# su1phurd/UAV-WRF-LES-PPO-LSTM

Hardware: AMD Instinct MI355X
Metric: env-steps/sec (rollout + GAE + 5-epoch PPO update), 4096 envs x 128 T per GPU, LSTM h=128 x1 (higher is better)
Workload: dtype f32

## Files before the change

uav-wrf-les-ppo-lstm_amd/csrc/common.h:

```cpp
#pragma once
#include <hip/hip_runtime.h>
#include <stdint.h>
#include <stdio.h>
#include <stdlib.h>
#include <string.h>
#include "../../include/uavppo.h"

struct uav_form_table {
    struct { const void* p; int v; } e[8];
    int next;
    void record(const void* p, int v) {
        for (auto& x : e)
            if (x.p == p) { x.v = v; return; }
        e[next] = {p, v};
        next = (next + 1) % 8;
    }
    int find(const void* p) const {
        for (auto& x : e)
            if (x.p == p) return x.v;
        return -1;
    }
};
struct uav_ctx {
    int device;
    int num_cu;
    void* ws;
    size_t ws_bytes;
    double* pow075;
    double* wave;
    double* ftab;
    int lstm_arith;
    unsigned debug;
    hipStream_t side[3];
    hipEvent_t side_ev[8];
    void* comm;
    int comm_rank, comm_world;
    uav_form_table dg_form;
    uav_form_table hslot_form;
};
static inline void uav_dg_record(uav_ctx* ctx, const void* p, int packed) { ctx->dg_form.record(p, packed); }
static inline int uav_dg_form(const uav_ctx* ctx, const void* p) { return ctx->dg_form.find(p); }

extern thread_local int g_uav_arith;
extern thread_local unsigned g_uav_debug;
static inline bool uav_want_f32_mfma() { return g_uav_arith == UAV_ARITH_F32_MFMA; }
static inline bool uav_want_bf16x6() { return g_uav_arith == UAV_ARITH_BF16X6; }
static inline bool uav_debug(unsigned bit) { return (g_uav_debug & bit) != 0; }
static inline void uav_enter(const struct uav_ctx* ctx);

static inline void uav_enter(const uav_ctx* ctx) {
    g_uav_arith = ctx->lstm_arith;
    g_uav_debug = ctx->debug;
}

void uav_set_error(const char* fmt, ...);

hipError_t uav_dyn_lds(const void* kernel, int bytes);

#define UAV_CHECK_HIP(expr)                                                          \
    do {                                                                             \
        hipError_t e_ = (expr);                                                      \
        if (e_ != hipSuccess) {                                                      \
            uav_set_error("%s:%d: %s -> %s", __FILE__, __LINE__, #expr, hipGetErrorString(e_)); \
            return 1;                                                                \
        }                                                                            \
    } while (0)

#define UAV_REQUIRE(cond, ...)                                                       \
    do {                                                                             \
        if (!(cond)) {                                                               \
            uav_set_error(__VA_ARGS__);                                              \
            return 2;                                                                \
        }                                                                            \
    } while (0)

#define UAV_LAUNCH_CHECK() UAV_CHECK_HIP(hipGetLastError())

static inline hipStream_t as_stream(uav_stream s) { return reinterpret_cast<hipStream_t>(s); }

constexpr int WAVE = 64;
// ... 85 lines not shown
    __device__ __forceinline__ static f32x4 mma(vec a, vec b, f32x4 c) { return __builtin_amdgcn_mfma_f32_16x16x32_bf16(a, b, c, 0, 0, 0); }
    template <class W>
    __device__ __forceinline__ static void gates_slab(f32x4 (&acc)[4], f32x4 (&)[4], W w, const vec (&a)[NP]) {
#pragma unroll
        for (int q = 0; q < 4; ++q) acc[q] = mma(w(q, 0), a[2], acc[q]);
#pragma unroll
        for (int q = 0; q < 4; ++q) acc[q] = mma(w(q, 1), a[1], acc[q]);
#pragma unroll
        for (int q = 0; q < 4; ++q) acc[q] = mma(w(q, 2), a[0], acc[q]);
#pragma unroll
        for (int q = 0; q < 4; ++q) acc[q] = mma(w(q, 0), a[1], acc[q]);
#pragma unroll
        for (int q = 0; q < 4; ++q) acc[q] = mma(w(q, 1), a[0], acc[q]);
#pragma unroll
        for (int q = 0; q < 4; ++q) acc[q] = mma(w(q, 0), a[0], acc[q]);
    }
    template <class W, class B>
    __device__ __forceinline__ static void head_slab(f32x4& ha, f32x4&, W w, B h) {
        ha = mma(w(0), h(2), ha);
        ha = mma(w(1), h(1), ha);
        ha = mma(w(2), h(0), ha);
        ha = mma(w(0), h(1), ha);
        ha = mma(w(1), h(0), ha);
        ha = mma(w(0), h(0), ha);
    }
    template <class V> __device__ __forceinline__ static V sum(V acc, V) { return acc; }
    template <class W>
    __device__ __forceinline__ static void tile_slab(f32x4& a0, f32x4& a1, W w, const vec (&b)[NP]) {
        a0 = mma(w(0), b[2], a0);
        a1 = mma(w(1), b[1], a1);
        a0 = mma(w(2), b[0], a0);
        a1 = mma(w(0), b[1], a1);
        a0 = mma(w(1), b[0], a0);
        a1 = mma(w(0), b[0], a1);
    }
    __device__ __forceinline__ static f32x4 tile_sum(f32x4 a0, f32x4 a1) { return a0 + a1; }
};

struct DgPack {
    static constexpr int H = 256, NS = 4 * H / 32;
    int N, T, NP, RT;
    __host__ __device__ DgPack(int n, int t) : N(n), T(t), NP((n + 63) / 64 * 64), RT(NP / 16) {}
    __host__ __device__ size_t step_halves() const { return (size_t)RT * NS * 1024; }
    __host__ __device__ size_t piece_bytes() const { return (size_t)T * step_halves() * 2; }
    __host__ __device__ size_t bytes() const { return piece_bytes() + 2 * (size_t)T * NP * sizeof(float); }
    __host__ __device__ unsigned short* pieces(void* base, int t) const { return (unsigned short*)base + (size_t)t * step_halves(); }
    __host__ __device__ const unsigned short* pieces(const void* base, int t) const { return (const unsigned short*)base + (size_t)t * step_halves(); }
    __host__ __device__ float* isc(void* base, int t) const { return (float*)((char*)base + piece_bytes()) + (size_t)t * NP; }
    __host__ __device__ const float* isc(const void* base, int t) const { return (const float*)((const char*)base + piece_bytes()) + (size_t)t * NP; }
    __host__ __device__ float* iscm(void* base, int t) const { return isc(base, T) + (size_t)t * NP; }
    __host__ __device__ const float* iscm(const void* base, int t) const { return isc(base, T) + (size_t)t * NP; }
};

__device__ __forceinline__ double wave_sum(double v) {
#pragma unroll
    for (int o = 32; o > 0; o >>= 1) v += __shfl_down(v, o, 64);
    return v;
}
__device__ __forceinline__ float wave_sum(float v) {
#pragma unroll
    for (int o = 32; o > 0; o >>= 1) v += __shfl_down(v, o, 64);
    return v;
}
__device__ __forceinline__ float wave_allsum(float v) {
#pragma unroll
    for (int o = 32; o > 0; o >>= 1) v += __shfl_xor(v, o, 64);
    return v;
}
template <typename T>
__device__ __forceinline__ T block256_sum(T v, T* sm) {
    v = wave_sum(v);
    const int lane = threadIdx.x & 63, w = threadIdx.x >> 6;
    if (lane == 0) sm[w] = v;
    __syncthreads();
    T r = T(0);
    if (threadIdx.x == 0) r = ((sm[0] + sm[1]) + sm[2]) + sm[3];
    __syncthreads();
    return r;
}
```

uav-wrf-les-ppo-lstm_amd/csrc/ctx.hip:

```cpp
#include <stdarg.h>
#include <mutex>
#include <set>
#include <utility>
#include "common.h"

static thread_local char g_err[512] = "";
thread_local int g_uav_arith = 0;
thread_local unsigned g_uav_debug = 0;
int env_init_tables(uav_ctx* ctx);

void uav_set_error(const char* fmt, ...) {
    va_list ap;
    va_start(ap, fmt);
    vsnprintf(g_err, sizeof(g_err), fmt, ap);
    va_end(ap);
}

hipError_t uav_dyn_lds(const void* kernel, int bytes) {
    static std::mutex mu;
    static std::set<std::pair<int, const void*>> done;
    int dev = 0;
    hipError_t e = hipGetDevice(&dev);
    if (e != hipSuccess) return e;
    std::lock_guard<std::mutex> lock(mu);
    if (done.count({dev, kernel})) return hipSuccess;
    e = hipFuncSetAttribute(kernel, hipFuncAttributeMaxDynamicSharedMemorySize, bytes);
    if (e == hipSuccess) done.insert({dev, kernel});
    return e;
}

extern "C" {

int uav_abi_version(void) { return UAV_ABI_VERSION; }
const char* uav_last_error(void) { return g_err; }

int uav_create(uav_ctx** out, int device, size_t ws_bytes) {
    UAV_REQUIRE(out != nullptr, "uav_create: out is NULL");
    UAV_REQUIRE(ws_bytes >= (1u << 20), "uav_create: ws_bytes must be >= 1 MiB");
    UAV_CHECK_HIP(hipSetDevice(device));
    hipDeviceProp_t prop;
    UAV_CHECK_HIP(hipGetDeviceProperties(&prop, device));
    UAV_REQUIRE(strncmp(prop.gcnArchName, "gfx950", 6) == 0,
                "libuavppo is built for gfx950 (MI355X) only; device %d is %s", device, prop.gcnArchName);
    uav_ctx* c = new uav_ctx();
    c->device = device;
    c->num_cu = prop.multiProcessorCount;
    c->ws_bytes = ws_bytes;
    c->pow075 = nullptr;
    c->wave = nullptr;
    c->ftab = nullptr;
    c->comm = nullptr;
    c->comm_rank = -1;
    c->comm_world = 0;
    c->lstm_arith = getenv("UAV_LSTM_F32_MFMA") ? UAV_ARITH_F32_MFMA : (getenv("UAV_LSTM_BF16X6") ? UAV_ARITH_BF16X6 : UAV_ARITH_FP16X3);
    c->debug = (getenv("UAV_LSTM_STEP_F32") ? UAV_DEBUG_STEP_F32 : 0u) | (getenv("UAV_LSTM_X_F32") ? UAV_DEBUG_X_F32 : 0u) |
               (getenv("UAV_LSTM_DG_F32") ? UAV_DEBUG_DG_F32 : 0u);
    if (hipMalloc(&c->ws, ws_bytes) != hipSuccess) {
        (void)hipFree(c->ws);
        delete c;
        uav_set_error("uav_create: hipMalloc(%zu) failed", ws_bytes);
        return 1;
    }
    if (env_init_tables(c) != 0) {
        (void)hipFree(c->ws);
        (void)hipFree(c->pow075);
        (void)hipFree(c->wave);
        (void)hipFree(c->ftab);
        delete c;
        return 1;
    }
    *out = c;
    return 0;
}

int uav_set_lstm_arith(uav_ctx* ctx, int mode) {
    UAV_REQUIRE(ctx && mode >= UAV_ARITH_FP16X3 && mode <= UAV_ARITH_F32_MFMA, "uav_set_lstm_arith: bad argument");
    ctx->lstm_arith = mode;
    return 0;
}
int uav_get_lstm_arith(const uav_ctx* ctx) { return ctx ? ctx->lstm_arith : -1; }

int uav_set_debug_flags(uav_ctx* ctx, unsigned flags) {
    UAV_REQUIRE(ctx && (flags & ~(UAV_DEBUG_STEP_F32 | UAV_DEBUG_X_F32 | UAV_DEBUG_DG_F32 | UAV_DEBUG_GEMM_TN_OFF)) == 0, "uav_set_debug_flags: bad argument");
    ctx->debug = flags;
    return 0;
}

void uav_destroy(uav_ctx* ctx) {
    if (!ctx) return;
    (void)uav_comm_destroy(ctx);
    for (auto& e : ctx->side_ev)
        if (e) (void)hipEventDestroy(e);
    for (auto& s : ctx->side)
        if (s) (void)hipStreamDestroy(s);
    (void)hipFree(ctx->ws);
    (void)hipFree(ctx->pow075);
    (void)hipFree(ctx->wave);
    (void)hipFree(ctx->ftab);
    delete ctx;
}

}
```

uav-wrf-les-ppo-lstm_amd/csrc/gae.hip:

```cpp
#include "common.h"

__global__ __launch_bounds__(256) void gae_scan_kernel(const float* __restrict__ rew,
                                                       const float* __restrict__ val,
                                                       const float* __restrict__ done,
                                                       const float* __restrict__ last_val, int n_env,
                                                       int T, float gamma, float gl, int mode,
                                                       float* __restrict__ adv) {
#pragma clang fp contract(off)
    const int lane = threadIdx.x & 63;
    const int env = blockIdx.x * 4 + (threadIdx.x >> 6);
    if (env >= n_env) return;
    const size_t row = (size_t)env * T;
    const int nchunk = (T + 63) >> 6;
    float carry = 0.f;
    float v_right = 0.f, d_right = 0.f;
    for (int c = nchunk - 1; c >= 0; --c) {
        const int t = c * 64 + lane;
        const bool in = t < T;
        const float r = in ? rew[row + t] : 0.f;
        const float v = in ? val[row + t] : 0.f;
        const float d = in ? done[row + t] : 0.f;
        float v1 = __shfl_down(v, 1, 64);
        float d1 = __shfl_down(d, 1, 64);
        if (lane == 63) { v1 = v_right; d1 = d_right; }
        float a = 1.f, b = 0.f;
        if (in) {
            float nnt, nv;
            const bool last = (t == T - 1);
            if (mode == UAV_GAE_REFERENCE_EXACT) {
                nnt = 1.0f - (last ? d : d1);
                nv = (last ? v : v1) * nnt;
            } else {
                nnt = 1.0f - d;
                nv = (last ? (last_val ? last_val[env] : 0.f) : v1) * nnt;
            }
            b = (r + gamma * nv) - v;
            a = gl * nnt;
        }
#pragma unroll
        for (int o = 1; o < 64; o <<= 1) {
            const float a2 = __shfl_down(a, o, 64);
            const float b2 = __shfl_down(b, o, 64);
            if (lane + o < 64) {
                b = b + a * b2;
                a = a * a2;
            }
        }
        const float A = b + a * carry;
        if (in) adv[row + t] = A;
        carry = __shfl(A, 0, 64);
        v_right = __shfl(v, 0, 64);
        d_right = __shfl(d, 0, 64);
    }
}

constexpr int STATS_BLOCKS = 512;

__global__ __launch_bounds__(256) void adv_stats_partial(const float* __restrict__ x, int64_t n,
                                                         double* __restrict__ partial) {
    __shared__ double sm[4];
    double s = 0.0, q = 0.0;
    for (int64_t i = (int64_t)blockIdx.x * 256 + threadIdx.x; i < n; i += (int64_t)gridDim.x * 256) {
        const double v = (double)x[i];
        s += v;
        q += v * v;
    }
    s = block256_sum(s, sm);
    q = block256_sum(q, sm);
    if (threadIdx.x == 0) {
        partial[2 * blockIdx.x] = s;
        partial[2 * blockIdx.x + 1] = q;
    }
}

__global__ __launch_bounds__(256) void adv_stats_final(const double* __restrict__ partial, int nb,
                                                       int64_t n, double* __restrict__ stats3) {
    __shared__ double sm[4];
    double s = 0.0, q = 0.0;
    for (int i = threadIdx.x; i < nb; i += 256) {
        s += partial[2 * i];
        q += partial[2 * i + 1];
    }
    s = block256_sum(s, sm);
    q = block256_sum(q, sm);
    if (threadIdx.x == 0) {
        stats3[0] = s;
        stats3[1] = q;
        stats3[2] = (double)n;
    }
}

__global__ __launch_bounds__(256) void adv_normalise_kernel(const float* __restrict__ adv,
                                                            const float* __restrict__ val, int64_t n,
                                                            const double* __restrict__ stats3,
                                                            float* __restrict__ adv_out,
                                                            float* __restrict__ ret_out) {
#pragma clang fp contract(off)
    const double cnt = stats3[2];
    const double mean_d = stats3[0] / cnt;
    const double var = (stats3[1] - cnt * mean_d * mean_d) / (cnt - 1.0);
    const float mean = (float)mean_d;
    float sd = (float)sqrt(var > 0.0 ? var : (var == var ? 0.0 : var));
    if (sd < 1e-6f || sd != sd) sd = 1.0f;
    const float den = sd + 1e-6f;
    for (int64_t i = (int64_t)blockIdx.x * 256 + threadIdx.x; i < n; i += (int64_t)gridDim.x * 256) {
        const float a = (adv[i] - mean) / den;
        adv_out[i] = a;
        ret_out[i] = a + val[i];
    }
}

__global__ __launch_bounds__(1024) void pack_success_kernel(const uint8_t* __restrict__ flags, int64_t n, int cap,
                                                            uint8_t* __restrict__ msg) {
    __shared__ int part[32];
    const int tid = threadIdx.x;
    int64_t per = (n + 1023) / 1024;
    per = (per + 15) / 16 * 16;
    const int64_t lo = (int64_t)tid * per, hi = (lo + per < n) ? lo + per : n;
    const bool vec = (reinterpret_cast<uintptr_t>(flags) & 15) == 0;
    auto visit = [&](auto&& f) {
        int64_t i = lo;
        if (vec)
            for (; i + 16 <= hi; i += 16) {
                const uint4 w = *reinterpret_cast<const uint4*>(flags + i);
                if ((w.x | w.y | w.z | w.w) == 0u) continue;
                const unsigned ww[4] = {w.x, w.y, w.z, w.w};
#pragma unroll
                for (int q = 0; q < 4; ++q)
#pragma unroll
                    for (int k = 0; k < 4; ++k) {
                        const uint8_t v = (ww[q] >> (8 * k)) & 255;
                        if (v) f(v);
                    }
            }
// ... 120 lines not shown
                    succ += __popcll(__ballot(i < n && chunk[k + i] != 0));
                }
                k += n;
                const double env_radius = s.radius;
                s.episodes += n; s.successes += succ;
                s.hist_len += n; s.win_succ += succ;
                const bool full = s.hist_len >= CUR_WINDOW;
                double rate = 0.0;
                if (full) {
                    rate = (double)s.win_succ / (double)s.hist_len;
                    s.bonus = s.bonus * pow(CUR_DECAY_FACTOR, 1.0 + rate);
                    s.bonus_is_f64 = 1.0;
                }
                s.bonus = fmax(s.bonus, 0.1);
                if (full) {
                    if (rate > CUR_SUCCESS_THRESHOLD)
                        s.radius = fmax(CUR_MIN_RADIUS, s.radius * pow(CUR_RADIUS_DECAY, 2.0 + 3.0 * (rate - CUR_SUCCESS_THRESHOLD)));
                    else if (rate < 0.25)
                        s.radius = fmin(CUR_INITIAL_RADIUS, s.radius * 1.1);
                    const double d = s.radius - env_radius;
                    if (fabs(d) > 5.0) s.radius = env_radius + 5.0 * (d > 0.0 ? 1.0 : (d < 0.0 ? -1.0 : 0.0));
                    s.hist_len = 0; s.win_succ = 0;
                }
            }
            __syncthreads();
            if (lane == 0) sh = s;
        }
    }
    __syncthreads();
    if (lane == 0) *st = sh;
}

extern "C" {

int uav_gae(uav_ctx* ctx, const float* rew, const float* val, const float* done,
            const float* last_val, int n_env, int horizon, float gamma, float lam, int mode,
            float* adv, uav_stream stream) {
    UAV_REQUIRE(ctx && rew && val && done && adv, "uav_gae: NULL argument");
    UAV_REQUIRE(n_env > 0 && horizon > 0, "uav_gae: n_env=%d horizon=%d", n_env, horizon);
    UAV_REQUIRE(mode == UAV_GAE_REFERENCE_EXACT || mode == UAV_GAE_STANDARD, "uav_gae: mode %d", mode);
    const float gl = (float)((double)gamma * (double)lam);
    const int blocks = (n_env + 3) / 4;
    hipLaunchKernelGGL(gae_scan_kernel, dim3(blocks), dim3(256), 0, as_stream(stream), rew, val, done,
                       last_val, n_env, horizon, gamma, gl, mode, adv);
    UAV_LAUNCH_CHECK();
    return 0;
}

int uav_adv_stats(uav_ctx* ctx, const float* adv, int64_t n, double* stats3, uav_stream stream) {
    UAV_REQUIRE(ctx && adv && stats3 && n > 0, "uav_adv_stats: bad argument");
    int nb = (int)((n + 1023) / 1024);
    if (nb > STATS_BLOCKS) nb = STATS_BLOCKS;
    double* partial = (double*)ctx->ws;
    hipLaunchKernelGGL(adv_stats_partial, dim3(nb), dim3(256), 0, as_stream(stream), adv, n, partial);
    hipLaunchKernelGGL(adv_stats_final, dim3(1), dim3(256), 0, as_stream(stream), partial, nb, n, stats3);
    UAV_LAUNCH_CHECK();
    return 0;
}

int uav_adv_normalise(uav_ctx* ctx, const float* adv, const float* val, int64_t n,
                      const double* stats3, float* adv_out, float* ret_out, uav_stream stream) {
    UAV_REQUIRE(ctx && adv && val && stats3 && adv_out && ret_out && n > 0, "uav_adv_normalise: bad argument");
    int nb = (int)((n + 1023) / 1024);
    if (nb > 2048) nb = 2048;
    hipLaunchKernelGGL(adv_normalise_kernel, dim3(nb), dim3(256), 0, as_stream(stream), adv, val, n, stats3,
                       adv_out, ret_out);
    UAV_LAUNCH_CHECK();
    return 0;
}


int uav_episode_rows(uav_ctx* ctx, const float* rew, const float* info, const uint8_t* flags, int n_env, int T, int env_offset,
                     double* carry, double* rows, int cap, int32_t* count, uav_stream stream) {
    UAV_REQUIRE(ctx && rew && info && flags && carry && rows && count && n_env > 0 && T > 0 && cap > 0, "uav_episode_rows: bad argument");
    hipLaunchKernelGGL(episode_rows_kernel, dim3((n_env + 63) / 64), dim3(64), 0, as_stream(stream), rew, info, flags, n_env, T, env_offset,
                       carry, rows, cap, count);
    UAV_LAUNCH_CHECK();
    return 0;
}

size_t uav_curriculum_state_bytes(void) { return sizeof(CurriculumState); }

int uav_curriculum_init(uav_ctx* ctx, void* state, double radius, double bonus, int bonus_is_f64, uav_stream stream) {
    UAV_REQUIRE(ctx && state && radius > 0.0, "uav_curriculum_init: bad argument");
    hipLaunchKernelGGL(curriculum_init_kernel, dim3(1), dim3(64), 0, as_stream(stream), (CurriculumState*)state, radius, bonus, bonus_is_f64);
    UAV_LAUNCH_CHECK();
    return 0;
}

int uav_curriculum_update(uav_ctx* ctx, void* state, const uint8_t* msgs, int world, int cap, uav_stream stream) {
    UAV_REQUIRE(ctx && state && msgs && world > 0 && cap > 0, "uav_curriculum_update: bad argument");
    hipLaunchKernelGGL(curriculum_update_kernel, dim3(1), dim3(64), 0, as_stream(stream), (CurriculumState*)state, msgs, world, cap);
    UAV_LAUNCH_CHECK();
    return 0;
}

int uav_pack_success_bits(uav_ctx* ctx, const uint8_t* flags, int64_t n, int cap, uint8_t* msg, uav_stream stream) {
    UAV_REQUIRE(ctx && flags && msg && n > 0 && cap > 0, "uav_pack_success_bits: bad argument");
    hipLaunchKernelGGL(pack_success_kernel, dim3(1), dim3(1024), 0, as_stream(stream), flags, n, cap, msg);
    UAV_LAUNCH_CHECK();
    return 0;
}

}
```

uav-wrf-les-ppo-lstm_amd/csrc/loss.hip:

```cpp
#include "common.h"
#include "philox.h"

#include "loss_core.h"

template <int A>
__device__ __forceinline__ void loss_block_epilogue(const LossAcc& a, const float* s_db, double* partial) {
    __shared__ double sm[4];
    const double s_pl = block256_sum(a.pl, sm), s_vl = block256_sum(a.vl, sm);
    const double s_en = block256_sum(a.en, sm), s_nan = block256_sum(a.nan, sm);
    double dbs[A + 1];
#pragma unroll
    for (int k = 0; k <= A; ++k) dbs[k] = block256_sum((double)s_db[k], sm);
    if (threadIdx.x == 0) {
        double* pp = partial + (size_t)LOSS_PSTRIDE * blockIdx.x;
        pp[0] = s_pl; pp[1] = s_vl; pp[2] = s_en; pp[3] = s_nan;
#pragma unroll
        for (int k = 0; k <= A; ++k) pp[4 + k] = dbs[k];
    }
}

template <int A>
__global__ __launch_bounds__(256) void ppo_loss_kernel(
    const float* __restrict__ logits, const float* __restrict__ value, const int32_t* __restrict__ act,
    const float* __restrict__ logp_old, const float* __restrict__ adv, const float* __restrict__ ret,
    const float* __restrict__ val_old, int64_t n, float inv_n, float clip, float beta,
    double* __restrict__ partial, float* __restrict__ dlogits, float* __restrict__ dvalue, int ldl, int ldv) {
    LossAcc acc{0.0, 0.0, 0.0, 0.0};
    float s_db[A + 1];
#pragma unroll
    for (int k = 0; k <= A; ++k) s_db[k] = 0.f;
    for (int64_t i = (int64_t)blockIdx.x * 256 + threadIdx.x; i < n; i += (int64_t)gridDim.x * 256) {
        float z[A], dz[A];
#pragma unroll
        for (int k = 0; k < A; ++k) z[k] = logits[i * ldl + k];
        const float dV = ppo_sample<A>(z, value[i * ldv], act[i], logp_old[i], adv[i], ret[i], val_old[i], inv_n, clip,
                                       beta, acc, dz);
        dvalue[i * ldv] = dV;
        s_db[A] += dV;
#pragma unroll
        for (int k = 0; k < A; ++k) {
            dlogits[i * ldl + k] = dz[k];
            s_db[k] += dz[k];
        }
    }
    loss_block_epilogue<A>(acc, s_db, partial);
}

typedef float f32x4_l __attribute__((ext_vector_type(4)));
template <int A, int H>
__global__ __launch_bounds__(256) void ppo_loss_from_y_kernel(
    const float* __restrict__ y, const float* __restrict__ w_head, const float* __restrict__ b_head,
    const int32_t* __restrict__ act, const float* __restrict__ logp_old, const float* __restrict__ adv,
    const float* __restrict__ ret, const float* __restrict__ val_old, int64_t n, float inv_n, float clip, float beta,
    double* __restrict__ partial, float* __restrict__ dheads) {
    constexpr int KS = H / 4, SEG = KS + 4, S = 4 * SEG + 8, NH = A + 1;
    __shared__ __attribute__((aligned(16))) float wbuf[16 * S];
    __shared__ __attribute__((aligned(16))) float ybuf[4][16 * S];
    __shared__ float hd[4][64 * 9];
    const int lane = threadIdx.x & 63, w = threadIdx.x >> 6, j = lane & 15, kq = lane >> 4;
    for (int idx = threadIdx.x; idx < 16 * H; idx += 256) {
        const int hdx = idx / H, uu = idx % H;
        wbuf[hdx * S + (uu / KS) * SEG + (uu % KS)] = (hdx < NH) ? w_head[(size_t)hdx * H + uu] : 0.f;
    }
    __syncthreads();
    LossAcc acc{0.0, 0.0, 0.0, 0.0};
    float s_db[A + 1];
#pragma unroll
    for (int k = 0; k <= A; ++k) s_db[k] = 0.f;
    float bh[NH];
#pragma unroll
    for (int k = 0; k < NH; ++k) bh[k] = b_head[k];
    const int64_t ntile = (n + 255) / 256;
    for (int64_t tile = blockIdx.x; tile < ntile; tile += gridDim.x) {
        const int64_t row0 = tile * 256 + w * 64;
        f32x4_l c4[4];
#pragma unroll
        for (int mi = 0; mi < 4; ++mi) {
            __builtin_amdgcn_wave_barrier();
#pragma unroll
            for (int i = 0; i < H / 16; ++i) {
                const int idx = i * 64 + lane, row = idx / (H / 4), c = idx % (H / 4);
                const int64_t r = row0 + 16 * mi + row;
                const float4 v = *reinterpret_cast<const float4*>(y + (r < n ? r : n - 1) * H + 4 * c);
                *reinterpret_cast<float4*>(&ybuf[w][row * S + ((4 * c) / KS) * SEG + (4 * c) % KS]) = v;
            }
            __builtin_amdgcn_s_waitcnt(0xc07f);
            __builtin_amdgcn_wave_barrier();
            const float* yr = &ybuf[w][j * S + kq * SEG];
            f32x4_l a0 = {0.f, 0.f, 0.f, 0.f}, a1 = a0;
            const float* wr = wbuf + j * S + kq * SEG;
#pragma unroll
            for (int s = 0; s < KS; s += 4) {
                const float4 av = *reinterpret_cast<const float4*>(yr + s);
                const float4 bv = *reinterpret_cast<const float4*>(wr + s);
                a0 = __builtin_amdgcn_mfma_f32_16x16x4f32(av.x, bv.x, a0, 0, 0, 0);
                a1 = __builtin_amdgcn_mfma_f32_16x16x4f32(av.y, bv.y, a1, 0, 0, 0);
                a0 = __builtin_amdgcn_mfma_f32_16x16x4f32(av.z, bv.z, a0, 0, 0, 0);
                a1 = __builtin_amdgcn_mfma_f32_16x16x4f32(av.w, bv.w, a1, 0, 0, 0);
// ... 69 lines not shown
    const int a = sample_categorical<A>(z, p, u ? &u[i] : nullptr, seed, counter, index_offset + i, forced ? &forced[i] : nullptr, qa, bad);
    if (bad) atomicAdd(nan_count, 1);
    if (probs_out) {
#pragma unroll
        for (int k = 0; k < A; ++k) probs_out[i * A + k] = p[k];
    }
    act_out[i] = a;
    const float lp = logf(fminf(fmaxf(qa, F32_EPS), 1.0f - F32_EPS));
    if (logp_out) logp_out[i] = lp;
    if (act_buf) {
        act_buf[i * T + t] = a;
        logp_buf[i * T + t] = lp;
        val_buf[i * T + t] = logits[i * stride + A];
    }
}

__global__ __launch_bounds__(256) void store_transition_kernel(int n, int T, int t, float* __restrict__ keep,
                                                               const float* __restrict__ rew, const float* __restrict__ done,
                                                               const uint8_t* __restrict__ flags, float* __restrict__ keep_buf,
                                                               float* __restrict__ rew_buf, float* __restrict__ done_buf,
                                                               uint8_t* __restrict__ flags_buf) {
    const int i = blockIdx.x * 256 + threadIdx.x;
    if (i >= n) return;
    const int64_t o = (int64_t)i * T + t;
    const float d = done[i];
    keep_buf[o] = keep[i];
    rew_buf[o] = rew[i];
    done_buf[o] = d;
    flags_buf[o] = flags[i];
    keep[i] = 1.0f - d;
}

int launch_loss_final(double* partial, int nb, int n_heads, double* loss_sums, float* dhead_bias, hipStream_t st) {
    hipLaunchKernelGGL(loss_final_kernel, dim3(1), dim3(1024), 0, st, partial, nb, n_heads, loss_sums, dhead_bias);
    UAV_LAUNCH_CHECK();
    return 0;
}

extern "C" {

int uav_ppo_loss(uav_ctx* ctx, const float* logits, const float* value, const int32_t* act,
                 const float* logp_old, const float* adv, const float* ret, const float* val_old,
                 int64_t n, int n_act, float inv_n, float clip, float ent_beta, double* loss_sums,
                 float* dlogits, float* dvalue, float* dhead_bias, uav_stream stream) {
    UAV_REQUIRE(ctx && logits && act && logp_old && adv && ret && val_old && loss_sums && dlogits,
                "uav_ppo_loss: NULL argument");
    UAV_REQUIRE((value == nullptr) == (dvalue == nullptr), "uav_ppo_loss: value and dvalue must both be NULL (packed) or both given");
    const int ldl = value ? n_act : n_act + 1, ldv = value ? 1 : n_act + 1;
    if (!value) { value = logits + n_act; dvalue = dlogits + n_act; }
    UAV_REQUIRE(n > 0, "uav_ppo_loss: n=%lld", (long long)n);
    int nb = (int)((n + 255) / 256);
    if (nb > LOSS_BLOCKS) nb = LOSS_BLOCKS;
    double* partial = (double*)ctx->ws;
#define LAUNCH_LOSS(A_)                                                                                  \
    hipLaunchKernelGGL(ppo_loss_kernel<A_>, dim3(nb), dim3(256), 0, as_stream(stream), logits, value,   \
                       act, logp_old, adv, ret, val_old, n, inv_n, clip, ent_beta, partial, dlogits, dvalue, ldl, ldv)
    switch (n_act) {
        case 2: LAUNCH_LOSS(2); break;
        case 3: LAUNCH_LOSS(3); break;
        case 4: LAUNCH_LOSS(4); break;
        case 5: LAUNCH_LOSS(5); break;
        case 6: LAUNCH_LOSS(6); break;
        case 8: LAUNCH_LOSS(8); break;
        default: UAV_REQUIRE(false, "uav_ppo_loss: n_act=%d unsupported", n_act);
    }
#undef LAUNCH_LOSS
    hipLaunchKernelGGL(loss_final_kernel, dim3(1), dim3(1024), 0, as_stream(stream), partial, nb, n_act + 1, loss_sums,
                       dhead_bias);
    UAV_LAUNCH_CHECK();
    return 0;
}

int uav_ppo_loss_from_y(uav_ctx* ctx, const float* y, const float* w_head, const float* b_head, const int32_t* act,
                         const float* logp_old, const float* adv, const float* ret, const float* val_old, int64_t n,
                         int hidden, int n_act, float inv_n, float clip, float ent_beta, double* loss_sums, float* dheads,
                         float* dhead_bias, uav_stream stream) {
    UAV_REQUIRE(ctx && y && w_head && b_head && act && logp_old && adv && ret && val_old && loss_sums && dheads,
                "uav_ppo_loss_from_y: NULL argument");
    UAV_REQUIRE(n > 0 && n_act == 5, "uav_ppo_loss_from_y: n=%lld n_act=%d (5 actions supported)", (long long)n, n_act);
    int nb = (int)((n + 255) / 256);
    if (nb > LOSS_BLOCKS) nb = LOSS_BLOCKS;
    double* partial = (double*)ctx->ws;
#define LAUNCH_LY(H_)                                                                                             \
    hipLaunchKernelGGL((ppo_loss_from_y_kernel<5, H_>), dim3(nb), dim3(256), 0, as_stream(stream), y, w_head, b_head, \
                       act, logp_old, adv, ret, val_old, n, inv_n, clip, ent_beta, partial, dheads)
    switch (hidden) {
        case 64: LAUNCH_LY(64); break;
        case 128: LAUNCH_LY(128); break;
        case 256: LAUNCH_LY(256); break;
        default: UAV_REQUIRE(false, "uav_ppo_loss_from_y: hidden=%d unsupported (64/128/256)", hidden);
    }
#undef LAUNCH_LY
    hipLaunchKernelGGL(loss_final_kernel, dim3(1), dim3(1024), 0, as_stream(stream), partial, nb, n_act + 1, loss_sums,
                       dhead_bias);
    UAV_LAUNCH_CHECK();
    return 0;
}

int uav_policy_sample(uav_ctx* ctx, const float* logits, int64_t n, int n_act, const float* u,
                      uint64_t seed, uint64_t counter, int64_t index_offset, const int32_t* forced_act, int32_t* act_out,
                      float* logp_out, float* probs_out, int32_t* nan_count, uav_stream stream) {
    UAV_REQUIRE(ctx && logits && act_out && logp_out && nan_count && n > 0, "uav_policy_sample: bad argument");
    const int nb = (int)((n + 255) / 256);
#define LAUNCH_S(A_)                                                                                      \
    hipLaunchKernelGGL(policy_sample_kernel<A_>, dim3(nb), dim3(256), 0, as_stream(stream), logits, n, u, \
                       seed, counter, index_offset, forced_act, act_out, logp_out, probs_out, nan_count)
    switch (n_act) {
        case 2: LAUNCH_S(2); break;
        case 3: LAUNCH_S(3); break;
        case 4: LAUNCH_S(4); break;
        case 5: LAUNCH_S(5); break;
        case 6: LAUNCH_S(6); break;
        case 8: LAUNCH_S(8); break;
        default: UAV_REQUIRE(false, "uav_policy_sample: n_act=%d unsupported", n_act);
    }
#undef LAUNCH_S
    UAV_LAUNCH_CHECK();
    return 0;
}

int uav_policy_sample_at(uav_ctx* ctx, const float* heads, int64_t heads_stride, int64_t n, int n_act, uint64_t seed,
// ... 37 lines not shown
```

uav-wrf-les-ppo-lstm_amd/csrc/wgrad.hip:

```cpp
#include <stdlib.h>
#include <type_traits>
#include "common.h"

typedef float f32x4 __attribute__((ext_vector_type(4)));

constexpr int KC = 16;

template <int H>
struct WG {
    static constexpr int NW = H / 16;
    static constexpr int NT_ = H / 16 + 1;
    static constexpr int NC = H + 16;
    static constexpr int SG = 4 * H + 16;
    static constexpr int SB = H + 16;
    static constexpr int SY = H + 16;
    static constexpr int SD = 48;
    static constexpr int BUF = KC * (SG + SB + SY + SD);
    static constexpr size_t LDS = 2 * BUF * sizeof(float);
    static constexpr size_t SLAB = (size_t)4 * H * NC + 16 * H;
};

template <int H>
__global__ __launch_bounds__(H * 4) void lstm_wgrad_kernel(
    const float* __restrict__ dgates, const float* __restrict__ y, const float* __restrict__ keep,
// ... 419 lines not shown
    commit_b(0);
    load_b(1);
    split_pair(0, 0);
    lds_barrier();
    WX_PROF_DECL;
    for (int sl = 0; sl < nslab; ++sl) {
        const int buf = sl & 1;
        WX_PROF_MARK(0);
        mfma_pair(buf, 0, sl);
        WX_PROF_DEP(acc[0][NT_ - 1]); WX_PROF_DEP(acc[1][NT_ - 1]); WX_PROF_MARK(2);
        commit_b(buf ^ 1);
        if constexpr (!P::LOADS_BETWEEN_TILES) load_b(sl + 2);
        WX_PROF_MARK(5);
        split_pair(sl, 1);
        WX_PROF_DEP(ap[0][0]); WX_PROF_DEP(ap[1][NP - 1]); WX_PROF_MARK(3);
        mfma_pair(buf, 1, sl);
        WX_PROF_DEP(acc[2][NT_ - 1]); WX_PROF_DEP(acc[3][NT_ - 1]); WX_PROF_MARK(4);
        if (!late) { lds_barrier(); WX_PROF_MARK(7); }
        split_pair(sl + 1, 0);
        WX_PROF_DEP(ap[0][0]); WX_PROF_DEP(ap[1][NP - 1]); WX_PROF_MARK(1);
        if (late) { lds_barrier(); WX_PROF_MARK(7); }
    }
    WX_PROF_FLUSH();
    float* slab = slabs + (size_t)blockIdx.x * WG<H>::SLAB;
#pragma unroll
    for (int mi = 0; mi < 4; ++mi)
#pragma unroll
        for (int r = 0; r < 4; ++r) {
            const float usc = pol.row_unscale(mi, r, kq);
#pragma unroll
            for (int ni = 0; ni < NT_; ++ni)
                slab[(size_t)(64 * w + 32 * (mi >> 1) + 2 * (4 * kq + r) + (mi & 1)) * G::NC + 16 * ni + j] =
                    acc[mi][ni][r] * (ni == NT_ - 1 ? usc * (P::BSCALE / P::XSCALE) : usc);
        }
#pragma unroll
    for (int r = 0; r < 4; ++r) slab[(size_t)4 * H * G::NC + (size_t)(4 * kq + r) * H + 16 * w + j] = acch[r];
}

template <int H, bool HEADS>
__global__ __launch_bounds__(H * 4) void lstm_wgrad_x6_kernel(
    const float* __restrict__ dgates, const float* __restrict__ y, const float* __restrict__ keep,
    const float* __restrict__ h0, const float* __restrict__ x, int I, const float* __restrict__ dheads, int NH,
    int N, int T, int rows_per_block, float* __restrict__ slabs) {
    lstm_wgrad_split<H, HEADS, WgBf16x6>(dgates, y, keep, h0, x, I, dheads, NH, N, T, rows_per_block, slabs);
}
template <int H, bool HEADS>
__global__ __launch_bounds__(H * 4) void lstm_wgrad_h3_kernel(
    const float* __restrict__ dgates, const float* __restrict__ y, const float* __restrict__ keep,
    const float* __restrict__ h0, const float* __restrict__ x, int I, const float* __restrict__ dheads, int NH,
    int N, int T, int rows_per_block, float* __restrict__ slabs) {
    lstm_wgrad_split<H, HEADS, WgF16x3>(dgates, y, keep, h0, x, I, dheads, NH, N, T, rows_per_block, slabs);
}

template <int H>
__global__ __launch_bounds__(256) void wgrad_reduce_kernel(const float* __restrict__ slabs, int nb, int I, int NH,
                                                           float* __restrict__ dw_ih, float* __restrict__ dw_hh,
                                                           float* __restrict__ db, float* __restrict__ db_hh,
                                                           float* __restrict__ dw_head) {
    using G = WG<H>;
    const size_t o = (size_t)blockIdx.x * 256 + threadIdx.x;
    if (o >= G::SLAB) return;
    float p8[8] = {0.f, 0.f, 0.f, 0.f, 0.f, 0.f, 0.f, 0.f};
    int b = 0;
    for (; b + 8 <= nb; b += 8)
#pragma unroll
        for (int k = 0; k < 8; ++k) p8[k] += slabs[(size_t)(b + k) * G::SLAB + o];
    for (; b < nb; ++b) p8[0] += slabs[(size_t)b * G::SLAB + o];
    const float s = ((p8[0] + p8[1]) + (p8[2] + p8[3])) + ((p8[4] + p8[5]) + (p8[6] + p8[7]));
    const size_t gsz = (size_t)4 * H * G::NC;
    if (o < gsz) {
        const int m = (int)(o / G::NC), c = (int)(o % G::NC);
        if (c < H) dw_hh[(size_t)m * H + c] = s;
        else if (c - H < I) dw_ih[(size_t)m * I + (c - H)] = s;
        else if (c - H == 6) {
            db[m] = s;
            if (db_hh) db_hh[m] = s;
        }
    } else if (dw_head) {
        const int a = (int)((o - gsz) / H), uu = (int)((o - gsz) % H);
        if (a < NH) dw_head[(size_t)a * H + uu] = s;
    }
}

template <class P, int H, bool HEADS>
static constexpr auto wgrad_split_kernel() {
    if constexpr (std::is_same<P, WgF16x3>::value) return &lstm_wgrad_h3_kernel<H, HEADS>;
    else return &lstm_wgrad_x6_kernel<H, HEADS>;
}

template <class P, int H>
static int launch_wgrad_split(const float* dgates, const float* y, const float* keep, const float* h0, const float* x, int I,
                              const float* dheads, int NH, int N, int T, int nb, int rpb, float* slabs, hipStream_t st) {
    const auto kern = dheads ? wgrad_split_kernel<P, H, true>() : wgrad_split_kernel<P, H, false>();
    const size_t lds = WGS<H, P>::LDS;
    UAV_CHECK_HIP(uav_dyn_lds(reinterpret_cast<const void*>(kern), (int)lds));
    hipLaunchKernelGGL(kern, dim3(nb), dim3(H * 4), lds, st, dgates, y, keep, h0, x, I, dheads, NH, N, T, rpb, slabs);
    return 0;
}

template <int H>
static int launch_wgrad(uav_ctx* ctx, const float* dgates, const float* y, const float* keep, const float* h0,
                        const float* x, int I, const float* dheads, int NH, int N, int T,
                        float* dw_ih, float* dw_hh, float* db, float* db_hh, float* dw_head, hipStream_t st) {
    using G = WG<H>;
    const int64_t NTr = (int64_t)N * T;
    int nb = ctx->num_cu;
    const int64_t max_nb = (int64_t)(ctx->ws_bytes / (G::SLAB * sizeof(float)));
    if (nb > max_nb) nb = (int)max_nb;
    UAV_REQUIRE(nb >= 1, "uav_lstm_wgrad: workspace too small for one slab");
    int64_t rpb = (NTr + nb - 1) / nb;
    rpb = (rpb + KC - 1) / KC * KC;
    nb = (int)((NTr + rpb - 1) / rpb);
    float* slabs = (float*)ctx->ws;
    {
        int64_t rpx = (NTr + nb - 1) / nb;
        rpx = (rpx + KS6 - 1) / KS6 * KS6;
        const int nbx = (int)((NTr + rpx - 1) / rpx);
        const bool split_ok = (NTr % rpx == 0) && T >= 8 && I <= 6 && (!dheads || NH <= 8) && NTr * 4 * H < (1ll << 30) &&
                              !uav_want_f32_mfma();
        if (split_ok) {
            const int rc = uav_want_bf16x6()
                               ? launch_wgrad_split<WgBf16x6, H>(dgates, y, keep, h0, x, I, dheads, NH, N, T, nbx, (int)rpx, slabs, st)
                               : launch_wgrad_split<WgF16x3, H>(dgates, y, keep, h0, x, I, dheads, NH, N, T, nbx, (int)rpx, slabs, st);
            if (rc) return rc;
            hipLaunchKernelGGL((wgrad_reduce_kernel<H>), dim3((unsigned)((G::SLAB + 255) / 256)), dim3(256), 0, st, slabs,
                               nbx, I, NH, dw_ih, dw_hh, db, db_hh, dw_head);
            UAV_LAUNCH_CHECK();
            return 0;
        }
    }
    UAV_CHECK_HIP(uav_dyn_lds(reinterpret_cast<const void*>(&lstm_wgrad_kernel<H>), (int)G::LDS));
    hipLaunchKernelGGL((lstm_wgrad_kernel<H>), dim3(nb), dim3(H * 4), G::LDS, st, dgates, y, keep, h0, x, I, dheads, NH, N,
                       T, rpb, slabs);
    hipLaunchKernelGGL((wgrad_reduce_kernel<H>), dim3((unsigned)((G::SLAB + 255) / 256)), dim3(256), 0, st, slabs, nb, I,
                       NH, dw_ih, dw_hh, db, db_hh, dw_head);
    UAV_LAUNCH_CHECK();
    return 0;
}

int lstm_wgrad_fused(uav_ctx* ctx, const float* dgates, const float* y, const float* keep, const float* h0,
                     const float* x, int I, const float* dheads, int NH, int N, int T, int H,
                     float* dw_ih, float* dw_hh, float* db, float* db_hh, float* dw_head, hipStream_t st) {
    switch (H) {
        case 64: return launch_wgrad<64>(ctx, dgates, y, keep, h0, x, I, dheads, NH, N, T, dw_ih, dw_hh, db, db_hh, dw_head, st);
        case 128: return launch_wgrad<128>(ctx, dgates, y, keep, h0, x, I, dheads, NH, N, T, dw_ih, dw_hh, db, db_hh, dw_head, st);
    }
    uav_set_error("lstm_wgrad_fused: H=%d unsupported", H);
    return 2;
}
```

Measured before the change: 76.00 million.

## Fuse final reductions via last-block tickets, pack loss I/O, vectorize wgrad reduce

Merges the separate single-block finalize kernels for advantage stats and PPO loss into the partial-reduction kernels, using an atomic last-block ticket so one fewer launch is needed per call. The loss kernel also gains a packed float2 load/store path for contiguous logits+value rows and processes two samples per iteration to raise memory-level parallelism. The wgrad slab reduction now reads float4 and splits the slab dimension across 8 thread groups combined in LDS. This adds atomics, fences and a persistent ticket buffer, which must be reset correctly and cannot be shared by concurrent launches.

```diff
diff --git a/uav-wrf-les-ppo-lstm_amd/csrc/common.h b/uav-wrf-les-ppo-lstm_amd/csrc/common.h
--- a/uav-wrf-les-ppo-lstm_amd/csrc/common.h
+++ b/uav-wrf-les-ppo-lstm_amd/csrc/common.h
@@ -26,6 +26,7 @@
     int num_cu;
     void* ws;
     size_t ws_bytes;
+    unsigned* tickets;
     double* pow075;
     double* wave;
     double* ftab;
@@ -217,6 +218,26 @@
     __host__ __device__ const float* iscm(const void* base, int t) const { return isc(base, T) + (size_t)t * NP; }
 };
 
+enum { UAV_TICKET_LOSS = 0, UAV_TICKET_ADV_STATS = 1, UAV_TICKET_COUNT = 4 };
+__device__ __forceinline__ bool last_block_ticket(unsigned* ticket) {
+    __shared__ int s_last;
+    if (threadIdx.x == 0) {
+        __threadfence();
+        const unsigned t = atomicAdd(ticket, 1u);
+        const bool last = (t == gridDim.x - 1);
+        if (last) __hip_atomic_store(ticket, 0u, __ATOMIC_RELAXED, __HIP_MEMORY_SCOPE_AGENT);
+        s_last = last;
+    }
+    __syncthreads();
+    const bool last = s_last != 0;
+    if (last) __threadfence();
+    return last;
+}
+__device__ __forceinline__ double ld_partial(const double* p) {
+    return __builtin_bit_cast(double, __hip_atomic_load(reinterpret_cast<const unsigned long long*>(p), __ATOMIC_RELAXED,
+                                                        __HIP_MEMORY_SCOPE_AGENT));
+}
+
 __device__ __forceinline__ double wave_sum(double v) {
 #pragma unroll
     for (int o = 32; o > 0; o >>= 1) v += __shfl_down(v, o, 64);
diff --git a/uav-wrf-les-ppo-lstm_amd/csrc/ctx.hip b/uav-wrf-les-ppo-lstm_amd/csrc/ctx.hip
--- a/uav-wrf-les-ppo-lstm_amd/csrc/ctx.hip
+++ b/uav-wrf-les-ppo-lstm_amd/csrc/ctx.hip
@@ -46,6 +46,7 @@
     c->device = device;
     c->num_cu = prop.multiProcessorCount;
     c->ws_bytes = ws_bytes;
+    c->tickets = nullptr;
     c->pow075 = nullptr;
     c->wave = nullptr;
     c->ftab = nullptr;
@@ -61,7 +62,16 @@
         uav_set_error("uav_create: hipMalloc(%zu) failed", ws_bytes);
         return 1;
     }
+    if (hipMalloc(&c->tickets, UAV_TICKET_COUNT * sizeof(unsigned)) != hipSuccess ||
+        hipMemset(c->tickets, 0, UAV_TICKET_COUNT * sizeof(unsigned)) != hipSuccess || hipDeviceSynchronize() != hipSuccess) {
+        (void)hipFree(c->tickets);
+        (void)hipFree(c->ws);
+        delete c;
+        uav_set_error("uav_create: ticket allocation failed");
+        return 1;
+    }
     if (env_init_tables(c) != 0) {
+        (void)hipFree(c->tickets);
         (void)hipFree(c->ws);
         (void)hipFree(c->pow075);
         (void)hipFree(c->wave);
@@ -94,6 +104,7 @@
     for (auto& s : ctx->side)
         if (s) (void)hipStreamDestroy(s);
     (void)hipFree(ctx->ws);
+    (void)hipFree(ctx->tickets);
     (void)hipFree(ctx->pow075);
     (void)hipFree(ctx->wave);
     (void)hipFree(ctx->ftab);
diff --git a/uav-wrf-les-ppo-lstm_amd/csrc/gae.hip b/uav-wrf-les-ppo-lstm_amd/csrc/gae.hip
--- a/uav-wrf-les-ppo-lstm_amd/csrc/gae.hip
+++ b/uav-wrf-les-ppo-lstm_amd/csrc/gae.hip
@@ -56,8 +56,8 @@
 
 constexpr int STATS_BLOCKS = 512;
 
-__global__ __launch_bounds__(256) void adv_stats_partial(const float* __restrict__ x, int64_t n,
-                                                         double* __restrict__ partial) {
+__global__ __launch_bounds__(256) void adv_stats_kernel(const float* __restrict__ x, int64_t n, double* __restrict__ partial,
+                                                        unsigned* __restrict__ ticket, double* __restrict__ stats3) {
     __shared__ double sm[4];
     double s = 0.0, q = 0.0;
     for (int64_t i = (int64_t)blockIdx.x * 256 + threadIdx.x; i < n; i += (int64_t)gridDim.x * 256) {
@@ -71,15 +71,13 @@
         partial[2 * blockIdx.x] = s;
         partial[2 * blockIdx.x + 1] = q;
     }
-}
-
-__global__ __launch_bounds__(256) void adv_stats_final(const double* __restrict__ partial, int nb,
-                                                       int64_t n, double* __restrict__ stats3) {
-    __shared__ double sm[4];
-    double s = 0.0, q = 0.0;
+    if (!last_block_ticket(ticket)) return;
+    const int nb = (int)gridDim.x;
+    s = 0.0;
+    q = 0.0;
     for (int i = threadIdx.x; i < nb; i += 256) {
-        s += partial[2 * i];
-        q += partial[2 * i + 1];
+        s += ld_partial(partial + 2 * i);
+        q += ld_partial(partial + 2 * i + 1);
     }
     s = block256_sum(s, sm);
     q = block256_sum(q, sm);
@@ -306,8 +304,8 @@
     int nb = (int)((n + 1023) / 1024);
     if (nb > STATS_BLOCKS) nb = STATS_BLOCKS;
     double* partial = (double*)ctx->ws;
-    hipLaunchKernelGGL(adv_stats_partial, dim3(nb), dim3(256), 0, as_stream(stream), adv, n, partial);
-    hipLaunchKernelGGL(adv_stats_final, dim3(1), dim3(256), 0, as_stream(stream), partial, nb, n, stats3);
+    hipLaunchKernelGGL(adv_stats_kernel, dim3(nb), dim3(256), 0, as_stream(stream), adv, n, partial,
+                       ctx->tickets + UAV_TICKET_ADV_STATS, stats3);
     UAV_LAUNCH_CHECK();
     return 0;
 }
diff --git a/uav-wrf-les-ppo-lstm_amd/csrc/loss.hip b/uav-wrf-les-ppo-lstm_amd/csrc/loss.hip
--- a/uav-wrf-les-ppo-lstm_amd/csrc/loss.hip
+++ b/uav-wrf-les-ppo-lstm_amd/csrc/loss.hip
@@ -19,31 +19,116 @@
     }
 }
 
+template <int NH>
+__device__ __forceinline__ void loss_final_in_block(const double* partial, int nb, double* __restrict__ out4,
+                                                    float* __restrict__ dbias) {
+    __shared__ double smf[64][17];
+    const int c = threadIdx.x & 15, g0 = threadIdx.x >> 4;
+#pragma unroll
+    for (int q = 0; q < 4; ++q) {
+        const int g = g0 + 16 * q;
+        double s0 = 0.0, s1 = 0.0, s2 = 0.0, s3 = 0.0;
+        int i = g;
+        for (; i + 192 < nb; i += 256) {
+            const double v0 = ld_partial(partial + (size_t)LOSS_PSTRIDE * i + c);
+            const double v1 = ld_partial(partial + (size_t)LOSS_PSTRIDE * (i + 64) + c);
+            const double v2 = ld_partial(partial + (size_t)LOSS_PSTRIDE * (i + 128) + c);
+            const double v3 = ld_partial(partial + (size_t)LOSS_PSTRIDE * (i + 192) + c);
+            s0 += v0; s1 += v1; s2 += v2; s3 += v3;
+        }
+        for (; i < nb; i += 64) s0 += ld_partial(partial + (size_t)LOSS_PSTRIDE * i + c);
+        smf[g][c] = (s0 + s1) + (s2 + s3);
+    }
+    __syncthreads();
+    if (threadIdx.x < 4 + NH) {
+        double r = 0.0;
+#pragma unroll
+        for (int k = 0; k < 64; ++k) r += smf[k][threadIdx.x];
+        if (threadIdx.x < 4) out4[threadIdx.x] = r;
+        else if (dbias) dbias[threadIdx.x - 4] = (float)r;
+    }
+}
+
 template <int A>
+struct LossIn { float z[A], V, lpo, ad, R, vo; int a; };
+
+template <int A, bool PACKED>
+__device__ __forceinline__ void loss_load(LossIn<A>& s, int64_t i, const float* __restrict__ logits,
+                                          const float* __restrict__ value, const int32_t* __restrict__ act,
+                                          const float* __restrict__ logp_old, const float* __restrict__ adv,
+                                          const float* __restrict__ ret, const float* __restrict__ val_old, int ldl, int ldv) {
+    if constexpr (PACKED) {
+        static_assert((A + 1) % 2 == 0, "packed rows are read as 8-byte pairs");
+        const float2* row = reinterpret_cast<const float2*>(logits + i * (A + 1));
+        float h[A + 1];
+#pragma unroll
+        for (int k = 0; k < (A + 1) / 2; ++k) {
+            const float2 v = row[k];
+            h[2 * k] = v.x;
+            h[2 * k + 1] = v.y;
+        }
+#pragma unroll
+        for (int k = 0; k < A; ++k) s.z[k] = h[k];
+        s.V = h[A];
+    } else {
+#pragma unroll
+        for (int k = 0; k < A; ++k) s.z[k] = logits[i * ldl + k];
+        s.V = value[i * ldv];
+    }
+    s.a = act[i];
+    s.lpo = logp_old[i];
+    s.ad = adv[i];
+    s.R = ret[i];
+    s.vo = val_old[i];
+}
+
+template <int A, bool PACKED>
+__device__ __forceinline__ void loss_one(const LossIn<A>& s, int64_t i, float inv_n, float clip, float beta, LossAcc& acc,
+                                         float (&s_db)[A + 1], float* __restrict__ dlogits, float* __restrict__ dvalue, int ldl,
+                                         int ldv) {
+    float dz[A];
+    const float dV = ppo_sample<A>(s.z, s.V, s.a, s.lpo, s.ad, s.R, s.vo, inv_n, clip, beta, acc, dz);
+    if constexpr (PACKED) {
+        float2* row = reinterpret_cast<float2*>(dlogits + i * (A + 1));
+        float h[A + 1];
+#pragma unroll
+        for (int k = 0; k < A; ++k) h[k] = dz[k];
+        h[A] = dV;
+#pragma unroll
+        for (int k = 0; k < (A + 1) / 2; ++k) row[k] = make_float2(h[2 * k], h[2 * k + 1]);
+    } else {
+        dvalue[i * ldv] = dV;
+#pragma unroll
+        for (int k = 0; k < A; ++k) dlogits[i * ldl + k] = dz[k];
+    }
+    s_db[A] += dV;
+#pragma unroll
+    for (int k = 0; k < A; ++k) s_db[k] += dz[k];
+}
+
+template <int A, bool PACKED>
 __global__ __launch_bounds__(256) void ppo_loss_kernel(
     const float* __restrict__ logits, const float* __restrict__ value, const int32_t* __restrict__ act,
     const float* __restrict__ logp_old, const float* __restrict__ adv, const float* __restrict__ ret,
     const float* __restrict__ val_old, int64_t n, float inv_n, float clip, float beta,
-    double* __restrict__ partial, float* __restrict__ dlogits, float* __restrict__ dvalue, int ldl, int ldv) {
+    double* __restrict__ partial, float* __restrict__ dlogits, float* __restrict__ dvalue, int ldl, int ldv,
+    unsigned* __restrict__ ticket, double* __restrict__ loss_sums, float* __restrict__ dhead_bias) {
     LossAcc acc{0.0, 0.0, 0.0, 0.0};
     float s_db[A + 1];
 #pragma unroll
     for (int k = 0; k <= A; ++k) s_db[k] = 0.f;
-    for (int64_t i = (int64_t)blockIdx.x * 256 + threadIdx.x; i < n; i += (int64_t)gridDim.x * 256) {
-        float z[A], dz[A];
-#pragma unroll
-        for (int k = 0; k < A; ++k) z[k] = logits[i * ldl + k];
-        const float dV = ppo_sample<A>(z, value[i * ldv], act[i], logp_old[i], adv[i], ret[i], val_old[i], inv_n, clip,
-                                       beta, acc, dz);
-        dvalue[i * ldv] = dV;
-        s_db[A] += dV;
-#pragma unroll
-        for (int k = 0; k < A; ++k) {
-            dlogits[i * ldl + k] = dz[k];
-            s_db[k] += dz[k];
-        }
+    const int64_t stride = (int64_t)gridDim.x * 256;
+    for (int64_t i = (int64_t)blockIdx.x * 256 + threadIdx.x; i < n; i += 2 * stride) {
+        const bool two = i + stride < n;
+        const int64_t i2 = two ? i + stride : i;
+        LossIn<A> s1, s2;
+        loss_load<A, PACKED>(s1, i, logits, value, act, logp_old, adv, ret, val_old, ldl, ldv);
+        loss_load<A, PACKED>(s2, i2, logits, value, act, logp_old, adv, ret, val_old, ldl, ldv);
+        loss_one<A, PACKED>(s1, i, inv_n, clip, beta, acc, s_db, dlogits, dvalue, ldl, ldv);
+        if (two) loss_one<A, PACKED>(s2, i2, inv_n, clip, beta, acc, s_db, dlogits, dvalue, ldl, ldv);
     }
     loss_block_epilogue<A>(acc, s_db, partial);
+    if (last_block_ticket(ticket)) loss_final_in_block<A + 1>(partial, (int)gridDim.x, loss_sums, dhead_bias);
 }
 
 typedef float f32x4_l __attribute__((ext_vector_type(4)));
@@ -219,21 +304,26 @@
     int nb = (int)((n + 255) / 256);
     if (nb > LOSS_BLOCKS) nb = LOSS_BLOCKS;
     double* partial = (double*)ctx->ws;
-#define LAUNCH_LOSS(A_)                                                                                  \
-    hipLaunchKernelGGL(ppo_loss_kernel<A_>, dim3(nb), dim3(256), 0, as_stream(stream), logits, value,   \
-                       act, logp_old, adv, ret, val_old, n, inv_n, clip, ent_beta, partial, dlogits, dvalue, ldl, ldv)
+    const bool packed8 = (ldl == n_act + 1) && (ldv == n_act + 1) && ((reinterpret_cast<uintptr_t>(logits) | reinterpret_cast<uintptr_t>(dlogits)) & 7) == 0;
+    unsigned* ticket = ctx->tickets + UAV_TICKET_LOSS;
+#define LAUNCH_LOSS_(A_, P_)                                                                                 \
+    hipLaunchKernelGGL((ppo_loss_kernel<A_, P_>), dim3(nb), dim3(256), 0, as_stream(stream), logits, value, \
+                       act, logp_old, adv, ret, val_old, n, inv_n, clip, ent_beta, partial, dlogits, dvalue, ldl, ldv, ticket, \
+                       loss_sums, dhead_bias)
+#define LAUNCH_LOSS(A_) LAUNCH_LOSS_(A_, false)
+#define LAUNCH_LOSS_ODD(A_) do { if (packed8) LAUNCH_LOSS_(A_, true); else LAUNCH_LOSS_(A_, false); } while (0)
     switch (n_act) {
         case 2: LAUNCH_LOSS(2); break;
-        case 3: LAUNCH_LOSS(3); break;
+        case 3: LAUNCH_LOSS_ODD(3); break;
         case 4: LAUNCH_LOSS(4); break;
-        case 5: LAUNCH_LOSS(5); break;
+        case 5: LAUNCH_LOSS_ODD(5); break;
         case 6: LAUNCH_LOSS(6); break;
         case 8: LAUNCH_LOSS(8); break;
         default: UAV_REQUIRE(false, "uav_ppo_loss: n_act=%d unsupported", n_act);
     }
+#undef LAUNCH_LOSS_ODD
 #undef LAUNCH_LOSS
-    hipLaunchKernelGGL(loss_final_kernel, dim3(1), dim3(1024), 0, as_stream(stream), partial, nb, n_act + 1, loss_sums,
-                       dhead_bias);
+#undef LAUNCH_LOSS_
     UAV_LAUNCH_CHECK();
     return 0;
 }
diff --git a/uav-wrf-les-ppo-lstm_amd/csrc/wgrad.hip b/uav-wrf-les-ppo-lstm_amd/csrc/wgrad.hip
--- a/uav-wrf-les-ppo-lstm_amd/csrc/wgrad.hip
+++ b/uav-wrf-les-ppo-lstm_amd/csrc/wgrad.hip
@@ -495,21 +495,45 @@
     lstm_wgrad_split<H, HEADS, WgF16x3>(dgates, y, keep, h0, x, I, dheads, NH, N, T, rows_per_block, slabs);
 }
 
+constexpr int RQ = 128;
 template <int H>
 __global__ __launch_bounds__(256) void wgrad_reduce_kernel(const float* __restrict__ slabs, int nb, int I, int NH,
                                                            float* __restrict__ dw_ih, float* __restrict__ dw_hh,
                                                            float* __restrict__ db, float* __restrict__ db_hh,
                                                            float* __restrict__ dw_head) {
     using G = WG<H>;
-    const size_t o = (size_t)blockIdx.x * 256 + threadIdx.x;
-    if (o >= G::SLAB) return;
-    float p8[8] = {0.f, 0.f, 0.f, 0.f, 0.f, 0.f, 0.f, 0.f};
-    int b = 0;
-    for (; b + 8 <= nb; b += 8)
-#pragma unroll
-        for (int k = 0; k < 8; ++k) p8[k] += slabs[(size_t)(b + k) * G::SLAB + o];
-    for (; b < nb; ++b) p8[0] += slabs[(size_t)b * G::SLAB + o];
-    const float s = ((p8[0] + p8[1]) + (p8[2] + p8[3])) + ((p8[4] + p8[5]) + (p8[6] + p8[7]));
+    static_assert(G::SLAB % 4 == 0, "slabs are read as float4");
+    __shared__ __attribute__((aligned(16))) float sp[8][RQ + 4];
+    const int k = threadIdx.x >> 5, quad = threadIdx.x & 31;
+    const size_t o4 = (size_t)blockIdx.x * RQ + 4 * quad;
+    float4 p = make_float4(0.f, 0.f, 0.f, 0.f);
+    if (o4 < G::SLAB) {
+        const float* src = slabs + o4;
+        const int nb8 = nb & ~7;
+        int b = k;
+        for (; b + 56 < nb8; b += 64) {
+            float4 v[8];
+#pragma unroll
+            for (int u = 0; u < 8; ++u) v[u] = *reinterpret_cast<const float4*>(src + (size_t)(b + 8 * u) * G::SLAB);
+#pragma unroll
+            for (int u = 0; u < 8; ++u) { p.x += v[u].x; p.y += v[u].y; p.z += v[u].z; p.w += v[u].w; }
+        }
+        for (; b < nb8; b += 8) {
+            const float4 v = *reinterpret_cast<const float4*>(src + (size_t)b * G::SLAB);
+            p.x += v.x; p.y += v.y; p.z += v.z; p.w += v.w;
+        }
+        if (k == 0)
+            for (b = nb8; b < nb; ++b) {
+                const float4 v = *reinterpret_cast<const float4*>(src + (size_t)b * G::SLAB);
+                p.x += v.x; p.y += v.y; p.z += v.z; p.w += v.w;
+            }
+    }
+    *reinterpret_cast<float4*>(&sp[k][4 * quad]) = p;
+    __syncthreads();
+    const size_t o = (size_t)blockIdx.x * RQ + threadIdx.x;
+    if (threadIdx.x >= RQ || o >= G::SLAB) return;
+    const int e = threadIdx.x;
+    const float s = ((sp[0][e] + sp[1][e]) + (sp[2][e] + sp[3][e])) + ((sp[4][e] + sp[5][e]) + (sp[6][e] + sp[7][e]));
     const size_t gsz = (size_t)4 * H * G::NC;
     if (o < gsz) {
         const int m = (int)(o / G::NC), c = (int)(o % G::NC);
@@ -566,7 +590,7 @@
                                ? launch_wgrad_split<WgBf16x6, H>(dgates, y, keep, h0, x, I, dheads, NH, N, T, nbx, (int)rpx, slabs, st)
                                : launch_wgrad_split<WgF16x3, H>(dgates, y, keep, h0, x, I, dheads, NH, N, T, nbx, (int)rpx, slabs, st);
             if (rc) return rc;
-            hipLaunchKernelGGL((wgrad_reduce_kernel<H>), dim3((unsigned)((G::SLAB + 255) / 256)), dim3(256), 0, st, slabs,
+            hipLaunchKernelGGL((wgrad_reduce_kernel<H>), dim3((unsigned)((G::SLAB + RQ - 1) / RQ)), dim3(256), 0, st, slabs,
                                nbx, I, NH, dw_ih, dw_hh, db, db_hh, dw_head);
             UAV_LAUNCH_CHECK();
             return 0;
@@ -575,7 +599,7 @@
     UAV_CHECK_HIP(uav_dyn_lds(reinterpret_cast<const void*>(&lstm_wgrad_kernel<H>), (int)G::LDS));
     hipLaunchKernelGGL((lstm_wgrad_kernel<H>), dim3(nb), dim3(H * 4), G::LDS, st, dgates, y, keep, h0, x, I, dheads, NH, N,
                        T, rpb, slabs);
-    hipLaunchKernelGGL((wgrad_reduce_kernel<H>), dim3((unsigned)((G::SLAB + 255) / 256)), dim3(256), 0, st, slabs, nb, I,
+    hipLaunchKernelGGL((wgrad_reduce_kernel<H>), dim3((unsigned)((G::SLAB + RQ - 1) / RQ)), dim3(256), 0, st, slabs, nb, I,
                        NH, dw_ih, dw_hh, db, db_hh, dw_head);
     UAV_LAUNCH_CHECK();
     return 0;
```

Result: slower. 74.65 million (-1.8%).
